# DCASE-REPO/DESED_task

Measured on AMD Instinct MI355X. Metric: 10s-clips/sec CRNN mean-teacher train @batch48, higher is better.
Workload: dtype f32 (fp32 storage and accumulation; the dense contractions of the wide layers run as split-bf16 MFMA, 3 bf16 products per fp32 product, fp32-level accuracy; everything else exact f32)

## Files before the change

### desed_task_amd/_lib.py

```python
import ctypes
import os
import re

_HERE = os.path.dirname(os.path.abspath(__file__))
_HEADER = os.path.join(os.path.dirname(_HERE), "include", "sed_hip.h")
LIB_PATH = os.path.join(_HERE, "libsed_hip.so")

_CTYPES = {"int": ctypes.c_int, "float": ctypes.c_float, "double": ctypes.c_double, "long long": ctypes.c_longlong,
           "unsigned": ctypes.c_uint, "unsigned int": ctypes.c_uint}

ERRORS = {-1: "bad argument", -2: "kernel launch failed", -3: "unsupported configuration"}


def parse_header(path=_HEADER):
    text = open(path).read()
    text = re.sub(r"/\*.*?\*/", "", text, flags=re.S)
    protos = {}
    for m in re.finditer(r"\b(?:int|long long)\s+(sed_\w+)\s*\(([^)]*)\)\s*;", text):
        args = []
        for a in m.group(2).split(","):
            a = a.strip()
            if "*" in a:
                args.append(ctypes.c_void_p)
            else:
                ty = re.sub(r"\bconst\b", "", a).strip()
                ty = ty.rsplit(None, 1)[0].strip()
                args.append(_CTYPES[ty])
        protos[m.group(1)] = args
    return protos


def header_constants(path=_HEADER):
    return {m.group(1): int(m.group(2)) for m in re.finditer(r"^#define\s+(SED_\w+)\s+(\d+)\b", open(path).read(), re.M)}


class _Lib:
    def __init__(self, path, is_emulator=False):
        self.path = path
        self.is_emulator = is_emulator
        import torch
        self._dll = ctypes.CDLL(path)
        self.protos = parse_header()
        for name, argtypes in self.protos.items():
            fn = getattr(self._dll, name)
            fn.argtypes = argtypes
            fn.restype = ctypes.c_longlong if name.endswith("_floats") else ctypes.c_int

    def value(self, name, *args):
        return getattr(self._dll, name)(*args)

    def call(self, name, *args):
        rc = getattr(self._dll, name)(*args)
        if rc != 0:
            raise RuntimeError("%s failed: %s (rc=%d)" % (name, ERRORS.get(rc, "?"), rc))


_lib = None


def get():
    global _lib
    if _lib is None:
        if not os.path.exists(LIB_PATH):
            raise RuntimeError(
                "desed_task_amd: %s is missing -- build it with `python -m desed_task_amd.build` "
                "(hipcc --offload-arch=gfx950).  There is no CPU fallback." % LIB_PATH)
        _lib = _Lib(LIB_PATH)
    return _lib


def use_library(path, is_emulator=True):
    global _lib
    _lib = _Lib(path, is_emulator=is_emulator) if path is not None else None
    return _lib


TUNING_KEYS = {"glu_grid_cap": 0, "glu_bwd128_split": 1, "convb_ck": 2, "convb_mp": 3, "block0_nocenter": 4, "glu_fwd128": 5, "wgrad_narrow": 6, "wgrad_cap": 7, "attn_valu": 8, "wgrad_wide": 9, "gru_lds_kb": 10, "mel_taps_mem": 11, "convb_tpw": 12, "mel_wave": 13, "gemm_ntn": 14, "linear_tiles": 15}


_tuning = {}


def set_tuning(key, value):
    get().call("sed_set_tuning", TUNING_KEYS[key], int(value))
    _tuning[key] = int(value)


def get_tuning(key):
    return _tuning.get(key, 0)


def check_tensor(t, name="tensor"):
    lib = get()
    if lib.is_emulator:
        if t.is_cuda:
            raise RuntimeError("%s: emulator build bound but tensor is on the GPU" % name)
    elif not t.is_cuda:
        raise RuntimeError("%s must live on the MI355X (cuda) device: there is no CPU path" % name)
    if not t.is_contiguous():
        raise RuntimeError("%s must be contiguous" % name)


def stream_ptr(t):
    if t.is_cuda:
        import torch
        return torch.cuda.current_stream(t.device).cuda_stream
    return 0
```

### desed_task_amd/csrc/sed_common.h

```cpp
#pragma once

#ifdef SED_EMU
#include "hip_emu.h"
#else
#include <hip/hip_runtime.h>
#define SED_DYN_SMEM(name) extern __shared__ __attribute__((aligned(16))) char name[]
#define SED_LAUNCH(kern, grid, block, smem, stream, ...) \
    hipLaunchKernelGGL(kern, grid, block, smem, stream, __VA_ARGS__)
typedef float f32x16 __attribute__((ext_vector_type(16)));
typedef float f32x4 __attribute__((ext_vector_type(4)));
typedef short s16x8 __attribute__((ext_vector_type(8)));
#endif

#include <stdint.h>

#define SED_API extern "C" __attribute__((visibility("default")))

#define SED_MAX_SMEM(kern, bytes) \
    (void)hipFuncSetAttribute((const void*)(kern), hipFuncAttributeMaxDynamicSharedMemorySize, (int)(bytes))

__global__ __launch_bounds__(256) static void sed_zero4_kernel(float* p0, int n0, float* p1, int n1, float* p2, int n2, float* p3, int n3) {
    const int i = blockIdx.x * 256 + threadIdx.x;
    if (i < n0) p0[i] = 0.f;
    if (i < n1) p1[i] = 0.f;
    if (i < n2) p2[i] = 0.f;
    if (i < n3) p3[i] = 0.f;
}
static inline void sed_zero4(hipStream_t s, float* p0, int n0, float* p1, int n1, float* p2, int n2, float* p3, int n3) {
    int n = n0 > n1 ? n0 : n1;
    n = n > n2 ? n : n2;
    n = n > n3 ? n : n3;
    if (n <= 0) return;
    SED_LAUNCH(sed_zero4_kernel, dim3((n + 255) / 256), dim3(256), 0, s, p0, n0, p1, n1, p2, n2, p3, n3);
}

#define SED_OK 0
#define SED_ERR_ARG (-1)
#define SED_ERR_LAUNCH (-2)
#define SED_ERR_UNSUPPORTED (-3)

enum { SED_TUNE_GLU_GRID_CAP = 0, SED_TUNE_GLU_BWD128_SPLIT = 1, SED_TUNE_CONVB_CK = 2, SED_TUNE_CONVB_MP = 3, SED_TUNE_B0_NOCENTER = 4, SED_TUNE_GLU_FWD128 = 5, SED_TUNE_WGRAD_NARROW = 6, SED_TUNE_WGRAD_CAP = 7,
       SED_TUNE_ATTN_VALU = 8, SED_TUNE_WGRAD_WIDE = 9, SED_TUNE_GRU_LDS_KB = 10, SED_TUNE_MEL_TAPS_MEM = 11, SED_TUNE_CONVB_TPW = 12, SED_TUNE_MEL_WAVE = 13, SED_TUNE_GEMM_NTN = 14, SED_TUNE_LINEAR_TILES = 15, SED_TUNE_COUNT = 16 };
extern int sed_tuning[SED_TUNE_COUNT];

static inline int sed_check_launch() {
    hipError_t e = hipGetLastError();
    return e == hipSuccess ? SED_OK : SED_ERR_LAUNCH;
}

__device__ __forceinline__ f32x16 mfma32(float a, float b, f32x16 c) {
#ifdef SED_EMU
    return emu_mfma_32x32x2(a, b, c);
#else
    return __builtin_amdgcn_mfma_f32_32x32x2f32(a, b, c, 0, 0, 0);
#endif
}
__device__ __forceinline__ int mfma32_row(int r, int lane) { return (r & 3) + 8 * (r >> 2) + 4 * (lane >> 5); }

__device__ __forceinline__ f32x4 mfma16(float a, float b, f32x4 c) {
#ifdef SED_EMU
    return emu_mfma_16x16x4(a, b, c);
#else
    return __builtin_amdgcn_mfma_f32_16x16x4f32(a, b, c, 0, 0, 0);
#endif
}

__device__ __forceinline__ f32x16 mfma32_bf16(s16x8 a, s16x8 b, f32x16 c) {
#ifdef SED_EMU
    return emu_mfma_32x32x16_bf16(a, b, c);
#else
    typedef __bf16 bf16x8_t __attribute__((ext_vector_type(8)));
    return __builtin_amdgcn_mfma_f32_32x32x16_bf16(__builtin_bit_cast(bf16x8_t, a), __builtin_bit_cast(bf16x8_t, b), c, 0, 0, 0);
#endif
}
__device__ __forceinline__ f32x4 mfma16_bf16(s16x8 a, s16x8 b, f32x4 c) {
#ifdef SED_EMU
    return emu_mfma_16x16x32_bf16(a, b, c);
#else
    typedef __bf16 bf16x8_t __attribute__((ext_vector_type(8)));
    return __builtin_amdgcn_mfma_f32_16x16x32_bf16(__builtin_bit_cast(bf16x8_t, a), __builtin_bit_cast(bf16x8_t, b), c, 0, 0, 0);
#endif
}
__device__ __forceinline__ unsigned short f32_to_bf16(float x) {
    unsigned u = __float_as_uint(x);
    u += 0x7FFFu + ((u >> 16) & 1u);
    return (unsigned short)(u >> 16);
}
__device__ __forceinline__ float bf16_to_f32(unsigned short h) { return __uint_as_float(((unsigned)h) << 16); }
__device__ __forceinline__ void bf16_split(float x, unsigned short& hi, unsigned short& lo) {
    hi = f32_to_bf16(x);
    lo = f32_to_bf16(x - bf16_to_f32(hi));
}

__device__ __forceinline__ float sed_sadd(float a, float b) {
#ifdef SED_EMU
    return a + b;
#else
    float r;
    asm("v_add_f32 %0, %1, %2" : "=v"(r) : "v"(a), "v"(b));
    return r;
#endif
}

__device__ __forceinline__ float sed_sfma(float a, float b, float c) {
#ifdef SED_EMU
    return fmaf(a, b, c);
#else
    float r;
    asm("v_fma_f32 %0, %1, %2, %3" : "=v"(r) : "v"(a), "v"(b), "v"(c));
    return r;
#endif
}

__device__ __forceinline__ void sed_sched_fence() {
#ifndef SED_EMU
    __builtin_amdgcn_sched_barrier(0);
#endif
}

__device__ __forceinline__ unsigned sed_alignbit(unsigned hi, unsigned lo, unsigned shift) {
#ifdef SED_EMU
    return (unsigned)(((((unsigned long long)hi) << 32) | lo) >> shift);
#else
    return __builtin_amdgcn_alignbit(hi, lo, shift);
#endif
// ... 299 lines not shown
```

### desed_task_amd/csrc/sed_conv.hip

```cpp
#include "sed_common.h"

__global__ __launch_bounds__(256) void pack_weights_kernel(const float* __restrict__ W, float* __restrict__ Wf,
                                                           float* __restrict__ Wd, int COUT, int CIN) {
    const int i = blockIdx.x * 256 + threadIdx.x;
    if (i >= COUT * CIN * 9) return;
    const int b = i % 3, a = (i / 3) % 3, ci = (i / 9) % CIN, co = i / (9 * CIN);
    const float w = W[i];
    Wf[((a * 3 + b) * CIN + ci) * COUT + co] = w;
    if (Wd) Wd[(((2 - a) * 3 + (2 - b)) * COUT + co) * CIN + ci] = w;
}
SED_API int sed_conv_pack_weights(const float* W, float* Wf, float* Wd, int COUT, int CIN, void* stream) {
    const int n = COUT * CIN * 9;
    SED_LAUNCH(pack_weights_kernel, dim3((n + 255) / 256), dim3(256), 0, (hipStream_t)stream, W, Wf, Wd, COUT, CIN);
    return sed_check_launch();
}
struct PackJobs {
    const float* W[8];
    float* Wf[8];
    float* Wd[8];
    int cout[8], cin[8], start[9];
    int n;
};
__global__ __launch_bounds__(256) void pack_weights_multi_kernel(PackJobs jobs) {
    const int i = blockIdx.x * 256 + threadIdx.x;
    if (i >= jobs.start[jobs.n]) return;
    int j = 0;
#pragma unroll
    for (int q = 1; q < 8; ++q) j += (q < jobs.n && i >= jobs.start[q]) ? 1 : 0;
    const int e = i - jobs.start[j], COUT = jobs.cout[j], CIN = jobs.cin[j];
    const int b = e % 3, a = (e / 3) % 3, ci = (e / 9) % CIN, co = e / (9 * CIN);
    const float w = jobs.W[j][e];
    jobs.Wf[j][((a * 3 + b) * CIN + ci) * COUT + co] = w;
    if (jobs.Wd[j]) jobs.Wd[j][(((2 - a) * 3 + (2 - b)) * COUT + co) * CIN + ci] = w;
}
SED_API int sed_conv_pack_multi(int n, const void* const* W, void* const* Wf, void* const* Wd, const int* cout, const int* cin,
                                   void* stream) {
    if (n < 1 || n > 8) return SED_ERR_ARG;
    PackJobs jobs;
    int tot = 0;
    for (int j = 0; j < n; ++j) {
        jobs.W[j] = (const float*)W[j]; jobs.Wf[j] = (float*)Wf[j]; jobs.Wd[j] = Wd ? (float*)Wd[j] : nullptr;
        jobs.cout[j] = cout[j]; jobs.cin[j] = cin[j]; jobs.start[j] = tot;
        tot += cout[j] * cin[j] * 9;
    }
    for (int j = n; j < 8; ++j) { jobs.W[j] = nullptr; jobs.Wf[j] = nullptr; jobs.Wd[j] = nullptr; jobs.cout[j] = 0; jobs.cin[j] = 0; jobs.start[j] = tot; }
    jobs.start[n] = tot;
    jobs.start[8] = tot;
    jobs.n = n;
    SED_LAUNCH(pack_weights_multi_kernel, dim3((tot + 255) / 256), dim3(256), 0, (hipStream_t)stream, jobs);
    return sed_check_launch();
}

__global__ __launch_bounds__(1024) void wgrad_reduce_kernel(const float* __restrict__ parts, float* __restrict__ dW, int nparts,
                                                            int COUT, int CIN) {
    __shared__ float4 red[64][16];
    const int tid = threadIdx.x, col = tid & 15, grp = tid >> 4, G = blockDim.x >> 4;
    const int j = blockIdx.x * 64 + 4 * col;
    const int n = 9 * CIN * COUT;
    float4 acc = make_float4(0.f, 0.f, 0.f, 0.f);
    if (j < n) {
#pragma unroll 4
        for (int p = grp; p < nparts; p += G) {
            const float4 v = *(const float4*)(parts + (size_t)p * n + j);
            acc.x += v.x; acc.y += v.y; acc.z += v.z; acc.w += v.w;
        }
    }
    red[grp][col] = acc;
    __syncthreads();
    if (grp == 0 && j < n) {
        for (int g = 1; g < G; ++g) { const float4 v = red[g][col]; acc.x += v.x; acc.y += v.y; acc.z += v.z; acc.w += v.w; }
        const int co = j % COUT, ci = (j / COUT) % CIN, tap = j / (COUT * CIN);
        float* d = dW + ((size_t)co * CIN + ci) * 9 + tap;
        d[0] = acc.x; d[(size_t)CIN * 9] = acc.y; d[(size_t)2 * CIN * 9] = acc.z; d[(size_t)3 * CIN * 9] = acc.w;
    }
}
static inline int wgrad_parts(int CIN, int COUT, int B, int T, int F) {
    if (CIN <= 32) {
        const int TF = F >= 32 ? 32 : F, TR = 128 / TF;
        const int ntiles = B * ((T + TR - 1) / TR) * (F / TF);
        int cap = CIN <= 16 ? 1024 : 512;
        if (sed_tuning[SED_TUNE_WGRAD_CAP] > 0) cap = sed_tuning[SED_TUNE_WGRAD_CAP];
        return ntiles < cap ? ntiles : cap;
    }
    const int ntiles = (B * T * F + 63) / 64;
    return ntiles < 56 ? ntiles : 56;
}
static inline bool wgrad_row_ok(int CIN, int COUT, int F) {
    return F >= 8 && 64 % F == 0 && COUT == 128 && (CIN == 64 || CIN == 128);
}
static inline int wgrad_row_parts(int CIN, int B, int T, int F) {
    const int ntiles = (B * T * F + 63) / 64, cap = CIN == 64 ? 168 : 84;
    return ntiles < cap ? ntiles : cap;
}
SED_API long long sed_conv_wgrad_scratch_floats(int B, int T, int F, int CIN, int COUT) {
    int parts = wgrad_parts(CIN, COUT, B, T, F);
    if (wgrad_row_ok(CIN, COUT, F) && wgrad_row_parts(CIN, B, T, F) > parts) parts = wgrad_row_parts(CIN, B, T, F);
    return (long long)parts * 9 * CIN * COUT;
}

#define CONV_THREADS(COUT) ((COUT) >= 64 ? 512 : 256)

template <int CIN, int COUT, int TF, int MP = 128>
struct ConvCfg {
    static constexpr int TR = MP / TF;
    static constexpr int PW = TF + 2, PH = TR + 2, PP = PW * PH;
    static constexpr int CK = CIN < 32 ? CIN : 32;
    static constexpr int CKP = CK + 1;
    static constexpr int NCH = CIN / CK;
    static constexpr int NT = (COUT + 31) / 32;
    static constexpr int WM = MP / 32;
    static constexpr int THREADS = CONV_THREADS(COUT);
    static constexpr int WN = THREADS / 64 / WM;
    static constexpr int NTW = NT / WN;
    static_assert(NTW >= 1 && NTW * WN == NT, "wave split must tile COUT");
    static constexpr int WCH = CK * COUT;
    static constexpr int PATCH_F = (PP * CKP + 3) & ~3;
    static constexpr int SMEM = (PATCH_F + 2 * WCH) * 4;
};

template <int CIN, int COUT, int TF, bool STATS, int MP = 128>
__global__ __launch_bounds__(CONV_THREADS(COUT)) void conv3x3_kernel(const float* __restrict__ x, const float* __restrict__ Wp,
                                                      const float* __restrict__ bias, float* __restrict__ y,
                                                      float* __restrict__ partial, int B, int T, int F) {
    using Cfg = ConvCfg<CIN, COUT, TF, MP>;
    constexpr int TR = Cfg::TR, PW = Cfg::PW, PP = Cfg::PP, CK = Cfg::CK, CKP = Cfg::CKP, NCH = Cfg::NCH, NT = Cfg::NT,
                  WCH = Cfg::WCH, NTW = Cfg::NTW, THREADS = Cfg::THREADS, WM = Cfg::WM;
    SED_DYN_SMEM(smem);
    float* patch = (float*)smem;
    float* wbuf = patch + Cfg::PATCH_F;
    const int tid = threadIdx.x, lane = tid & 63, w = (tid >> 6) % WM, wn = (tid >> 6) / WM, lo = lane & 31, hi = lane >> 5;
    const int ftiles = F / TF, ttiles = (T + TR - 1) / TR;
    const int bid = blockIdx.x;
    const int ft = bid % ftiles, tt = (bid / ftiles) % ttiles, b = bid / (ftiles * ttiles);
    const int t0 = tt * TR, f0 = ft * TF;
    const int p = 32 * w + lo;
    const int abase = ((p / TF) * PW + (p % TF)) * CKP + hi;

    f32x16 acc[NTW];
#pragma unroll
    for (int nt = 0; nt < NTW; ++nt) acc[nt] = f32x16_zero();

    constexpr int WV = (WCH / 4 + THREADS - 1) / THREADS;
    float4 wreg[WV];

    for (int cc = 0; cc < NCH; ++cc) {
        constexpr int V = CK / 4;
        {
            constexpr int NLD = (PP * V + THREADS - 1) / THREADS;
            float4 ld[NLD];
#pragma unroll
            for (int u = 0; u < NLD; ++u) {
                const int idx = tid + THREADS * u;
                const int pix = idx / V, v = idx - pix * V;
                const int i = pix / PW, j = pix - i * PW;
                const int t = t0 - 1 + i, f = f0 - 1 + j;
                ld[u] = make_float4(0.f, 0.f, 0.f, 0.f);
                if (idx < PP * V && t >= 0 && t < T && f >= 0 && f < F)
                    ld[u] = *(const float4*)(x + (((size_t)b * T + t) * F + f) * CIN + cc * CK + 4 * v);
            }
#pragma unroll
            for (int u = 0; u < NLD; ++u) {
                const int idx = tid + THREADS * u;
                if (idx < PP * V) {
                    const int pix = idx / V, v = idx - pix * V;
                    float* d = patch + pix * CKP + 4 * v;
                    d[0] = ld[u].x; d[1] = ld[u].y; d[2] = ld[u].z; d[3] = ld[u].w;
                }
            }
        }
        {
            const float4* src = (const float4*)(Wp + ((size_t)0 * CIN + cc * CK) * COUT);
#pragma unroll
            for (int i = 0; i < WV; ++i) {
                const int idx = tid + THREADS * i;
                if (idx < WCH / 4) ((float4*)wbuf)[idx] = src[idx];
// ... 340 lines not shown
                const int idx = tid + 256 * u, r = idx / (COUT / 4), v = idx - r * (COUT / 4);
                *(float4*)(ds + r * COUT + 4 * v) = ldy[u];
            }
        }
        __syncthreads();
        constexpr int KS = KT / WK;
#pragma unroll 4
        for (int k = wk * KS; k < (wk + 1) * KS; k += 2) {
            float av[MT];
#pragma unroll
            for (int m = 0; m < MT; ++m) av[m] = (CIN >= 32 || lo < CIN) ? xs[(k + hi) * CIN + m * 32 + lo] : 0.f;
#pragma unroll
            for (int n = 0; n < NTW; ++n) {
                const int co = (wn * NTW + n) * 32 + lo;
                const float bv = (COUT >= 32 || lo < COUT) ? ds[(k + hi) * COUT + co] : 0.f;
#pragma unroll
                for (int m = 0; m < MT; ++m) acc[m][n] = mfma32(av[m], bv, acc[m][n]);
            }
        }
    }
    static_assert(WK == 1, "wide layers: every wave owns its output tiles");
    float* part = dWp + ((size_t)blockIdx.x * 9 + tap) * CIN * COUT;
#pragma unroll
    for (int m = 0; m < MT; ++m)
#pragma unroll
        for (int n = 0; n < NTW; ++n) {
            const int co = (wn * NTW + n) * 32 + lo;
#pragma unroll
            for (int r = 0; r < 16; ++r) {
                const int ci = m * 32 + mfma32_row(r, lane);
                if (ci < CIN && co < COUT) part[(size_t)ci * COUT + co] = acc[m][n][r];
            }
        }
}

template <int CIN, int COUT>
static int launch_wgrad(const float* x, const float* dy, float* dWp, int B, int T, int F, hipStream_t s) {
    using Cfg = WgCfg<CIN, COUT>;
    const int splits = wgrad_parts(CIN, COUT, B, T, F);
    SED_MAX_SMEM((conv_wgrad_kernel<CIN, COUT>), Cfg::SMEM);
    SED_LAUNCH((conv_wgrad_kernel<CIN, COUT>), dim3(splits, 9), dim3(256), Cfg::SMEM, s, x, dy, dWp, B, T, F);
    return sed_check_launch();
}

template <int CIN, int COUT, int NP = 3>
struct WgbCfg {
    static constexpr int PLANES = NP == 1 ? 1 : 2;
    static constexpr int KT = 64, RS = 64;
    static constexpr int MT = CIN / 32, NT = COUT / 32;
    static constexpr int WM = MT >= 4 ? 2 : 1, WN = 4 / WM;
    static constexpr int MTW = MT / WM, NTW = NT / WN;
    static constexpr int NBX = (KT / 4) * (CIN / 4) / 256, NBD = (KT / 4) * (COUT / 4) / 256;
    static constexpr int SMEM = PLANES * (CIN + COUT) * RS * 2;
    static_assert(NBX >= 1 && NBD >= 1 && MTW * WM == MT && NTW * WN == NT, "tile split");
};

template <bool LO = true>
__device__ __forceinline__ void wgb_store_row(float a, float b, float c, float d, unsigned short* __restrict__ hi_row,
                                              unsigned short* __restrict__ lo_row) {
    if constexpr (!LO) {
        *(uint2*)hi_row = make_uint2(bf16_round2(a, b), bf16_round2(c, d));
    } else {
    uint2 h, l;
    bf16_split2(a, b, h.x, l.x);
    bf16_split2(c, d, h.y, l.y);
    *(uint2*)hi_row = h;
    *(uint2*)lo_row = l;
    }
}
template <bool LO = true>
__device__ __forceinline__ void wgb_store_block(const float4 v0, const float4 v1, const float4 v2, const float4 v3,
                                                unsigned short* __restrict__ hi_plane, unsigned short* __restrict__ lo_plane,
                                                int cq, int pq, int RS) {
    const int r0 = 4 * cq, f0 = (r0 ^ cq) & 7;
    const int o0 = r0 * RS + 4 * (pq ^ (2 * f0)), o1 = (r0 + 1) * RS + 4 * (pq ^ (2 * (f0 ^ 1)));
    const int o2 = (r0 + 2) * RS + 4 * (pq ^ (2 * (f0 ^ 2))), o3 = (r0 + 3) * RS + 4 * (pq ^ (2 * (f0 ^ 3)));
    wgb_store_row<LO>(v0.x, v1.x, v2.x, v3.x, hi_plane + o0, lo_plane + o0);
    wgb_store_row<LO>(v0.y, v1.y, v2.y, v3.y, hi_plane + o1, lo_plane + o1);
    wgb_store_row<LO>(v0.z, v1.z, v2.z, v3.z, hi_plane + o2, lo_plane + o2);
    wgb_store_row<LO>(v0.w, v1.w, v2.w, v3.w, hi_plane + o3, lo_plane + o3);
}

template <int CIN, int COUT, class... ONE>
__global__ __launch_bounds__(256) void conv_wgrad_bf16_kernel(const float* __restrict__ x, const float* __restrict__ dy,
                                                              float* __restrict__ dWp, int B, int T, int F) {
    constexpr int NP = sed_np<ONE...>();
    using Cfg = WgbCfg<CIN, COUT, NP>;
    constexpr int KT = Cfg::KT, RS = Cfg::RS, WN = Cfg::WN, MTW = Cfg::MTW, NTW = Cfg::NTW, NBX = Cfg::NBX, NBD = Cfg::NBD;
    SED_DYN_SMEM(smem);
    unsigned short* xh = (unsigned short*)smem;
    unsigned short* xl = xh + (Cfg::PLANES - 1) * CIN * RS;
    unsigned short* dh = xl + CIN * RS;
    unsigned short* dl = dh + (Cfg::PLANES - 1) * COUT * RS;
    const int tid = threadIdx.x, lane = tid & 63, w = tid >> 6, lo = lane & 31, hi = lane >> 5;
    const int wn = w % WN, wm = w / WN;
    const int tap = blockIdx.y, da = tap / 3 - 1, db = tap % 3 - 1;
    const int npix = B * T * F;
    const int ntiles = (npix + KT - 1) / KT;
    const int fsh = 31 - __builtin_clz(F);

    f32x16 acc[MTW][NTW];
#pragma unroll
    for (int m = 0; m < MTW; ++m)
#pragma unroll
        for (int n = 0; n < NTW; ++n) acc[m][n] = f32x16_zero();

    float4 rx[NBX * 4], rd[NBD * 4];
    unsigned okx = 0, okd = 0;
    static_assert(NBX * 4 <= 32 && NBD * 4 <= 32, "validity masks");
    auto load_tile = [&](int tile) {
        const int p0 = tile * KT;
        okx = 0; okd = 0;
#pragma unroll
        for (int u = 0; u < NBX; ++u) {
            const int blk = tid + 256 * u, cq = (blk >> 1) % (CIN / 4), pq = (blk & 1) + 2 * ((blk >> 1) / (CIN / 4));
#pragma unroll
            for (int j = 0; j < 4; ++j) {
                const int p = p0 + 4 * pq + j, pc = p < npix ? p : 0;
                const int f = pc & (F - 1), tt = pc >> fsh, t = tt % T, bb = tt / T;
                const int t2 = t + da, f2 = f + db;
                const bool ok = p < npix && t2 >= 0 && t2 < T && f2 >= 0 && f2 < F;
                okx |= (ok ? 1u : 0u) << (4 * u + j);
                const int t2c = t2 < 0 ? 0 : (t2 >= T ? T - 1 : t2), f2c = f2 < 0 ? 0 : (f2 >= F ? F - 1 : f2);
                rx[4 * u + j] = *(const float4*)(x + (((size_t)bb * T + t2c) * F + f2c) * CIN + 4 * cq);
            }
        }
#pragma unroll
        for (int u = 0; u < NBD; ++u) {
            const int blk = tid + 256 * u, cq = (blk >> 1) % (COUT / 4), pq = (blk & 1) + 2 * ((blk >> 1) / (COUT / 4));
#pragma unroll
            for (int j = 0; j < 4; ++j) {
                const int p = p0 + 4 * pq + j;
                okd |= (p < npix ? 1u : 0u) << (4 * u + j);
                rd[4 * u + j] = *(const float4*)(dy + (size_t)(p < npix ? p : 0) * COUT + 4 * cq);
            }
        }
    };
    auto store_tile = [&]() {
#pragma unroll
        for (int i = 0; i < NBX * 4; ++i) if (!((okx >> i) & 1u)) rx[i] = make_float4(0.f, 0.f, 0.f, 0.f);
#pragma unroll
        for (int i = 0; i < NBD * 4; ++i) if (!((okd >> i) & 1u)) rd[i] = make_float4(0.f, 0.f, 0.f, 0.f);
#pragma unroll
        for (int u = 0; u < NBX; ++u) {
            const int blk = tid + 256 * u;
            wgb_store_block<NP != 1>(rx[4 * u], rx[4 * u + 1], rx[4 * u + 2], rx[4 * u + 3], xh, xl, (blk >> 1) % (CIN / 4),
                            (blk & 1) + 2 * ((blk >> 1) / (CIN / 4)), RS);
        }
#pragma unroll
        for (int u = 0; u < NBD; ++u) {
            const int blk = tid + 256 * u;
            wgb_store_block<NP != 1>(rd[4 * u], rd[4 * u + 1], rd[4 * u + 2], rd[4 * u + 3], dh, dl, (blk >> 1) % (COUT / 4),
                            (blk & 1) + 2 * ((blk >> 1) / (COUT / 4)), RS);
        }
    };

    int tile = blockIdx.x;
    if (tile < ntiles) load_tile(tile);
    for (; tile < ntiles; tile += gridDim.x) {
        __syncthreads();
        store_tile();
        __syncthreads();
        if (tile + (int)gridDim.x < ntiles) load_tile(tile + gridDim.x);
#pragma unroll
        for (int ks = 0; ks < KT / 16; ++ks) {
            const int oct = 2 * ks + hi;
            s16x8 a_hi[MTW], a_lo[MTW];
#pragma unroll
            for (int m = 0; m < MTW; ++m) {
                const int row = (wm * MTW + m) * 32 + lo;
                const int off = row * RS + 8 * (oct ^ ((row ^ (row >> 2)) & 7));
                a_hi[m] = *(const s16x8*)(xh + off);
                if constexpr (NP != 1) a_lo[m] = *(const s16x8*)(xl + off);
            }
#pragma unroll
            for (int n = 0; n < NTW; ++n) {
                const int row = (wn * NTW + n) * 32 + lo;
                const int off = row * RS + 8 * (oct ^ ((row ^ (row >> 2)) & 7));
                const s16x8 b_hi = *(const s16x8*)(dh + off);
                if constexpr (NP == 1) {
#pragma unroll
                    for (int m = 0; m < MTW; ++m) acc[m][n] = mfma32_bf16(a_hi[m], b_hi, acc[m][n]);
                    continue;
                }
                const s16x8 b_lo = *(const s16x8*)(dl + off);
#pragma unroll
                for (int m = 0; m < MTW; ++m) {
                    acc[m][n] = mfma32_bf16(a_lo[m], b_hi, acc[m][n]);
                    acc[m][n] = mfma32_bf16(a_hi[m], b_lo, acc[m][n]);
                    acc[m][n] = mfma32_bf16(a_hi[m], b_hi, acc[m][n]);
                }
            }
        }
    }
    float* part = dWp + ((size_t)blockIdx.x * 9 + tap) * CIN * COUT;
#pragma unroll
    for (int m = 0; m < MTW; ++m)
#pragma unroll
        for (int n = 0; n < NTW; ++n) {
            const int co = (wn * NTW + n) * 32 + lo;
#pragma unroll
            for (int r = 0; r < 16; ++r) part[(size_t)((wm * MTW + m) * 32 + mfma32_row(r, lane)) * COUT + co] = acc[m][n][r];
        }
}

template <int CIN, int COUT, int NP = 3>
static int launch_wgrad_bf16(const float* x, const float* dy, float* dWp, int B, int T, int F, hipStream_t s) {
    using Cfg = WgbCfg<CIN, COUT, NP>;
    const int splits = wgrad_parts(CIN, COUT, B, T, F);
    SED_MAX_SMEM((NP == 1 ? conv_wgrad_bf16_kernel<CIN, COUT, SedOneProduct> : conv_wgrad_bf16_kernel<CIN, COUT>), Cfg::SMEM);
    SED_LAUNCH((NP == 1 ? conv_wgrad_bf16_kernel<CIN, COUT, SedOneProduct> : conv_wgrad_bf16_kernel<CIN, COUT>), dim3(splits, 9), dim3(256), Cfg::SMEM, s, x, dy, dWp, B, T, F);
    return sed_check_launch();
}

template <int CIN, int COUT, int COH, int NP = 3>
struct WgrCfg {
    static constexpr int PLANES = NP == 1 ? 1 : 2;
    static constexpr int KT = 64, RS = 64;
    static constexpr int MT = CIN / 32, NT = COH / 32;
    static constexpr int WM = MT >= 4 ? 2 : 1, WN = 4 / WM;
    static constexpr int MTW = MT / WM, NTW = NT / WN;
    static constexpr int NBX = (KT / 4) * (CIN / 4) / 256, NBD = (KT / 4) * (COH / 4) / 256;
    static constexpr int SMEM = PLANES * (CIN + COH) * RS * 2;
    static_assert(NBX >= 1 && NBD >= 1 && MTW * WM == MT && NTW * WN == NT && MTW * NTW == 2, "tile split");
};
template <int CIN, int COUT, int COH, class... ONE>
__global__ __launch_bounds__(256) void conv_wgrad_bf16_row_kernel(const float* __restrict__ x, const float* __restrict__ dy,
                                                                  float* __restrict__ dWp, int B, int T, int F) {
    constexpr int NP = sed_np<ONE...>();
    using Cfg = WgrCfg<CIN, COUT, COH, NP>;
    constexpr int KT = Cfg::KT, RS = Cfg::RS, WN = Cfg::WN, MTW = Cfg::MTW, NTW = Cfg::NTW, NBX = Cfg::NBX, NBD = Cfg::NBD;
    SED_DYN_SMEM(smem);
    unsigned short* xh = (unsigned short*)smem;
    unsigned short* xl = xh + (Cfg::PLANES - 1) * CIN * RS;
    unsigned short* dh = xl + CIN * RS;
    unsigned short* dl = dh + (Cfg::PLANES - 1) * COH * RS;
    const int lane = threadIdx.x & 63, w = threadIdx.x >> 6;
    int tid = threadIdx.x, lo = lane & 31, hi = lane >> 5;
    const int wn = w % WN, wm = w / WN;
    const int da = (int)blockIdx.y - 1, co0 = blockIdx.z * COH;
    const int npix = B * T * F;
    const int ntiles = (npix + KT - 1) / KT;
    const int fsh = 31 - __builtin_clz(F);

    f32x16 acc[3][MTW][NTW];
#pragma unroll
    for (int t3 = 0; t3 < 3; ++t3)
#pragma unroll
        for (int m = 0; m < MTW; ++m)
#pragma unroll
            for (int n = 0; n < NTW; ++n) acc[t3][m][n] = f32x16_zero();

    float4 rx[NBX * 4], rd[NBD * 4];
    unsigned okm = 0;
    auto load_tile = [&](int tile) {
        const int p0 = tile * KT;
        okm = 0;
#pragma unroll
        for (int u = 0; u < NBX; ++u) {
            const int blk = tid + 256 * u, cq = (blk >> 1) % (CIN / 4), pq = (blk & 1) + 2 * ((blk >> 1) / (CIN / 4));
            const int pb = p0 + 4 * pq, pbc = pb < npix ? pb : 0, tt = pbc >> fsh, t = tt % T, bb = tt / T, t2 = t + da, f = pbc & (F - 1);
            const bool ok = pb < npix && t2 >= 0 && t2 < T;
            okm |= (ok ? 1u : 0u) << u;
            const float* src = x + (((size_t)bb * T + (t2 < 0 ? 0 : (t2 >= T ? T - 1 : t2))) * F + f) * CIN + 4 * cq;
#pragma unroll
            for (int j = 0; j < 4; ++j) rx[4 * u + j] = *(const float4*)(src + (size_t)j * CIN);
        }
#pragma unroll
        for (int u = 0; u < NBD; ++u) {
            const int blk = tid + 256 * u, cq = (blk >> 1) % (COH / 4), pq = (blk & 1) + 2 * ((blk >> 1) / (COH / 4));
            const int pb = p0 + 4 * pq;
            okm |= (pb < npix ? 1u : 0u) << (16 + u);
            const float* src = dy + (size_t)(pb < npix ? pb : 0) * COUT + co0 + 4 * cq;
#pragma unroll
            for (int j = 0; j < 4; ++j) rd[4 * u + j] = *(const float4*)(src + (size_t)j * COUT);
        }
    };
    auto store_tile = [&]() {
#pragma unroll
        for (int u = 0; u < NBX; ++u)
            if (!((okm >> u) & 1u)) {
#pragma unroll
                for (int j = 0; j < 4; ++j) rx[4 * u + j] = make_float4(0.f, 0.f, 0.f, 0.f);
            }
#pragma unroll
        for (int u = 0; u < NBD; ++u)
            if (!((okm >> (16 + u)) & 1u)) {
#pragma unroll
                for (int j = 0; j < 4; ++j) rd[4 * u + j] = make_float4(0.f, 0.f, 0.f, 0.f);
            }
#pragma unroll
        for (int u = 0; u < NBX; ++u) {
            const int blk = tid + 256 * u;
            wgb_store_block<NP != 1>(rx[4 * u], rx[4 * u + 1], rx[4 * u + 2], rx[4 * u + 3], xh, xl, (blk >> 1) % (CIN / 4),
                            (blk & 1) + 2 * ((blk >> 1) / (CIN / 4)), RS);
        }
#pragma unroll
        for (int u = 0; u < NBD; ++u) {
            const int blk = tid + 256 * u;
            wgb_store_block<NP != 1>(rd[4 * u], rd[4 * u + 1], rd[4 * u + 2], rd[4 * u + 3], dh, dl, (blk >> 1) % (COH / 4),
                            (blk & 1) + 2 * ((blk >> 1) / (COH / 4)), RS);
        }
    };
    auto shift_m1 = [](const uint4 c, unsigned prev3) {
        uint4 r;
        r.x = sed_alignbit(c.x, prev3, 16); r.y = sed_alignbit(c.y, c.x, 16); r.z = sed_alignbit(c.z, c.y, 16); r.w = sed_alignbit(c.w, c.z, 16);
        return r;
    };
    auto shift_p1 = [](const uint4 c, unsigned next0) {
        uint4 r;
        r.x = sed_alignbit(c.y, c.x, 16); r.y = sed_alignbit(c.z, c.y, 16); r.z = sed_alignbit(c.w, c.z, 16); r.w = sed_alignbit(next0, c.w, 16);
        return r;
    };

    int tile = blockIdx.x;
    if (tile < ntiles) load_tile(tile);
    for (; tile < ntiles; tile += gridDim.x) {
        sed_opaque(tid); sed_opaque(lo); sed_opaque(hi);
        __syncthreads();
        store_tile();
        __syncthreads();
        if (tile + (int)gridDim.x < ntiles) load_tile(tile + gridDim.x);
#pragma unroll
        for (int ks = 0; ks < KT / 16; ++ks) {
            const int oct = 2 * ks + hi;
            const bool first = ((8 * oct) & (F - 1)) == 0, last = ((8 * oct + 8) & (F - 1)) == 0;
            s16x8 a_hi[3][MTW], a_lo[3][MTW];
#pragma unroll
            for (int m = 0; m < MTW; ++m) {
                const int row = (wm * MTW + m) * 32 + lo, sw = (row ^ (row >> 2)) & 7;
                const int off = row * RS + 8 * (oct ^ sw);
                const int offp = row * RS + 8 * (((oct + 7) & 7) ^ sw) + 6, offn = row * RS + 8 * (((oct + 1) & 7) ^ sw);
                if constexpr (NP == 1) {
                    const uint4 ch = *(const uint4*)(xh + off);
                    const unsigned ph = first ? 0u : *(const unsigned*)(xh + offp), nh = last ? 0u : *(const unsigned*)(xh + offn);
                    a_hi[0][m] = __builtin_bit_cast(s16x8, shift_m1(ch, ph));
                    a_hi[1][m] = __builtin_bit_cast(s16x8, ch);
                    a_hi[2][m] = __builtin_bit_cast(s16x8, shift_p1(ch, nh));
                    continue;
                }
                const uint4 ch = *(const uint4*)(xh + off), cl = *(const uint4*)(xl + off);
                const unsigned ph = first ? 0u : *(const unsigned*)(xh + offp), pl = first ? 0u : *(const unsigned*)(xl + offp);
                const unsigned nh = last ? 0u : *(const unsigned*)(xh + offn), nl = last ? 0u : *(const unsigned*)(xl + offn);
                a_hi[0][m] = __builtin_bit_cast(s16x8, shift_m1(ch, ph)); a_lo[0][m] = __builtin_bit_cast(s16x8, shift_m1(cl, pl));
                a_hi[1][m] = __builtin_bit_cast(s16x8, ch);               a_lo[1][m] = __builtin_bit_cast(s16x8, cl);
                a_hi[2][m] = __builtin_bit_cast(s16x8, shift_p1(ch, nh)); a_lo[2][m] = __builtin_bit_cast(s16x8, shift_p1(cl, nl));
            }
#pragma unroll
            for (int n = 0; n < NTW; ++n) {
                const int row = (wn * NTW + n) * 32 + lo;
                const int off = row * RS + 8 * (oct ^ ((row ^ (row >> 2)) & 7));
                const s16x8 b_hi = *(const s16x8*)(dh + off);
                if constexpr (NP == 1) {
#pragma unroll
                    for (int t3 = 0; t3 < 3; ++t3)
#pragma unroll
                        for (int m = 0; m < MTW; ++m) acc[t3][m][n] = mfma32_bf16(a_hi[t3][m], b_hi, acc[t3][m][n]);
                    continue;
                }
                const s16x8 b_lo = *(const s16x8*)(dl + off);
#pragma unroll
                for (int t3 = 0; t3 < 3; ++t3)
#pragma unroll
                    for (int m = 0; m < MTW; ++m) {
                        acc[t3][m][n] = mfma32_bf16(a_lo[t3][m], b_hi, acc[t3][m][n]);
                        acc[t3][m][n] = mfma32_bf16(a_hi[t3][m], b_lo, acc[t3][m][n]);
                        acc[t3][m][n] = mfma32_bf16(a_hi[t3][m], b_hi, acc[t3][m][n]);
                    }
            }
        }
    }
#pragma unroll
    for (int t3 = 0; t3 < 3; ++t3) {
        float* part = dWp + ((size_t)blockIdx.x * 9 + 3 * (da + 1) + t3) * CIN * COUT;
#pragma unroll
        for (int m = 0; m < MTW; ++m)
#pragma unroll
            for (int n = 0; n < NTW; ++n) {
                const int co = co0 + (wn * NTW + n) * 32 + lo;
#pragma unroll
                for (int r = 0; r < 16; ++r) part[(size_t)((wm * MTW + m) * 32 + mfma32_row(r, lane)) * COUT + co] = acc[t3][m][n][r];
            }
    }
}
template <int CIN, int COUT, int COH, int NP = 3>
static int launch_wgrad_bf16_row(const float* x, const float* dy, float* dWp, int B, int T, int F, int splits, hipStream_t s) {
    using Cfg = WgrCfg<CIN, COUT, COH, NP>;
    SED_MAX_SMEM((NP == 1 ? conv_wgrad_bf16_row_kernel<CIN, COUT, COH, SedOneProduct> : conv_wgrad_bf16_row_kernel<CIN, COUT, COH>), Cfg::SMEM);
    SED_LAUNCH((NP == 1 ? conv_wgrad_bf16_row_kernel<CIN, COUT, COH, SedOneProduct> : conv_wgrad_bf16_row_kernel<CIN, COUT, COH>), dim3(splits, 3, COUT / COH), dim3(256), Cfg::SMEM, s, x, dy, dWp, B, T, F);
    return sed_check_launch();
}

template <int CIN, int COUT, int TF>
struct WgaCfg {
    static constexpr int TR = 128 / TF, PW = TF + 2, PH = TR + 2, PP = PW * PH;
    static constexpr int NT = COUT / 32, WN = NT >= 2 ? 2 : 1, WK = 4 / WN, NTW = NT / WN;
    static constexpr int SMEM = (PP * CIN + 128 * COUT) * 4;
};
template <int CIN, int COUT, int TF>
__global__ __launch_bounds__(256) void conv_wgrad_alltaps_kernel(const float* __restrict__ x, const float* __restrict__ dy,
                                                                 float* __restrict__ dWp, int B, int T, int F) {
    using Cfg = WgaCfg<CIN, COUT, TF>;
    constexpr int TR = Cfg::TR, PW = Cfg::PW, PP = Cfg::PP, WN = Cfg::WN, WK = Cfg::WK, NTW = Cfg::NTW;
    static_assert(CIN <= 32, "narrow layers only");
    SED_DYN_SMEM(smem);
    float* xs = (float*)smem;
    float* ds = xs + PP * CIN;
    const int tid = threadIdx.x, lane = tid & 63, w = tid >> 6, lo = lane & 31, hi = lane >> 5;
    const int wn = w % WN, wk = w / WN;
    const int ftiles = F / TF, ttiles = (T + TR - 1) / TR, ntiles = B * ttiles * ftiles;
    constexpr bool M16 = CIN == 16;
    constexpr int NT16 = COUT / 16, WK16 = 4;
    f32x16 acc[M16 ? 1 : 9][M16 ? 1 : NTW];
    f32x4 acc16[M16 ? 9 : 1][M16 ? NT16 : 1];
#pragma unroll
    for (int tp = 0; tp < (M16 ? 1 : 9); ++tp)
#pragma unroll
        for (int n = 0; n < (M16 ? 1 : NTW); ++n) acc[tp][n] = f32x16_zero();
#pragma unroll
    for (int tp = 0; tp < (M16 ? 9 : 1); ++tp)
#pragma unroll
        for (int n = 0; n < (M16 ? NT16 : 1); ++n) acc16[tp][n] = f32x4{0.f, 0.f, 0.f, 0.f};

    constexpr int NX = (PP * (CIN / 4) + 255) / 256, ND = 128 * (COUT / 4) / 256;
    float4 lx[NX], ldy[ND];
    auto load_tile = [&](int tile_) {
        const int ft = tile_ % ftiles, tt = (tile_ / ftiles) % ttiles, b = tile_ / (ftiles * ttiles);
        const int t0 = tt * TR, f0 = ft * TF;
#pragma unroll
        for (int u = 0; u < NX; ++u) {
            const int idx = tid + 256 * u, pix = idx / (CIN / 4), v = idx - pix * (CIN / 4);
            const int i = pix / PW, j = pix - i * PW;
            const int t = t0 - 1 + i, f = f0 - 1 + j;
            float4 val = make_float4(0.f, 0.f, 0.f, 0.f);
            if (idx < PP * (CIN / 4) && t >= 0 && t < T && f >= 0 && f < F)
                val = *(const float4*)(x + (((size_t)b * T + t) * F + f) * CIN + 4 * v);
            lx[u] = val;
        }
#pragma unroll
        for (int u = 0; u < ND; ++u) {
            const int idx = tid + 256 * u, p = idx / (COUT / 4), v = idx - p * (COUT / 4);
            const int t = t0 + p / TF, f = f0 + p % TF;
            float4 val = make_float4(0.f, 0.f, 0.f, 0.f);
            if (t < T) val = *(const float4*)(dy + (((size_t)b * T + t) * F + f) * COUT + 4 * v);
            ldy[u] = val;
        }
    };
    int tile = blockIdx.x;
    if (tile < ntiles) load_tile(tile);
    for (; tile < ntiles; tile += gridDim.x) {
        __syncthreads();
#pragma unroll
        for (int u = 0; u < NX; ++u) {
            const int idx = tid + 256 * u;
            if (idx < PP * (CIN / 4)) *(float4*)(xs + (idx / (CIN / 4)) * CIN + 4 * (idx % (CIN / 4))) = lx[u];
        }
#pragma unroll
        for (int u = 0; u < ND; ++u) {
            const int idx = tid + 256 * u;
            *(float4*)(ds + (idx / (COUT / 4)) * COUT + 4 * (idx % (COUT / 4))) = ldy[u];
        }
        __syncthreads();
        if (tile + (int)gridDim.x < ntiles) load_tile(tile + gridDim.x);
        if (M16) {
            constexpr int KS16 = 128 / WK16;
            const int i16 = lane & 15, g16 = lane >> 4;
#pragma unroll 2
            for (int k = w * KS16; k < (w + 1) * KS16; k += 4) {
                const int p = k + g16;
                const int pb = (p / TF) * PW + (p % TF);
                float bv16[NT16];
#pragma unroll
// ... 476 lines not shown
```

Before: 16690.

## Run two 256-thread groups per wide wgrad block and reduce accumulators in LDS

The wide-layer bf16 weight-gradient kernels now launch 512 threads, two independent 256-thread groups each with its own LDS planes, processing interleaved tiles. At the end the second group's accumulators are exchanged through LDS and summed by the first group before writing partials. The split counts are halved, so fewer per-split partial slabs need to be written and reduced, and the two groups can overlap loads and MFMA inside one block. In exchange the block uses twice the LDS and a larger block size, which may lower occupancy, and it adds an LDS reduction step. A new tuning knob overrides the split cap.

```diff
diff --git a/desed_task_amd/_lib.py b/desed_task_amd/_lib.py
--- a/desed_task_amd/_lib.py
+++ b/desed_task_amd/_lib.py
@@ -75,7 +75,7 @@
     return _lib
 
 
-TUNING_KEYS = {"glu_grid_cap": 0, "glu_bwd128_split": 1, "convb_ck": 2, "convb_mp": 3, "block0_nocenter": 4, "glu_fwd128": 5, "wgrad_narrow": 6, "wgrad_cap": 7, "attn_valu": 8, "wgrad_wide": 9, "gru_lds_kb": 10, "mel_taps_mem": 11, "convb_tpw": 12, "mel_wave": 13, "gemm_ntn": 14, "linear_tiles": 15}
+TUNING_KEYS = {"glu_grid_cap": 0, "glu_bwd128_split": 1, "convb_ck": 2, "convb_mp": 3, "block0_nocenter": 4, "glu_fwd128": 5, "wgrad_narrow": 6, "wgrad_cap": 7, "attn_valu": 8, "wgrad_wide": 9, "gru_lds_kb": 10, "mel_taps_mem": 11, "convb_tpw": 12, "mel_wave": 13, "gemm_ntn": 14, "linear_tiles": 15, "wgrad_wide_splits": 16}
 
 
 _tuning = {}
diff --git a/desed_task_amd/csrc/sed_common.h b/desed_task_amd/csrc/sed_common.h
--- a/desed_task_amd/csrc/sed_common.h
+++ b/desed_task_amd/csrc/sed_common.h
@@ -40,7 +40,7 @@
 #define SED_ERR_UNSUPPORTED (-3)
 
 enum { SED_TUNE_GLU_GRID_CAP = 0, SED_TUNE_GLU_BWD128_SPLIT = 1, SED_TUNE_CONVB_CK = 2, SED_TUNE_CONVB_MP = 3, SED_TUNE_B0_NOCENTER = 4, SED_TUNE_GLU_FWD128 = 5, SED_TUNE_WGRAD_NARROW = 6, SED_TUNE_WGRAD_CAP = 7,
-       SED_TUNE_ATTN_VALU = 8, SED_TUNE_WGRAD_WIDE = 9, SED_TUNE_GRU_LDS_KB = 10, SED_TUNE_MEL_TAPS_MEM = 11, SED_TUNE_CONVB_TPW = 12, SED_TUNE_MEL_WAVE = 13, SED_TUNE_GEMM_NTN = 14, SED_TUNE_LINEAR_TILES = 15, SED_TUNE_COUNT = 16 };
+       SED_TUNE_ATTN_VALU = 8, SED_TUNE_WGRAD_WIDE = 9, SED_TUNE_GRU_LDS_KB = 10, SED_TUNE_MEL_TAPS_MEM = 11, SED_TUNE_CONVB_TPW = 12, SED_TUNE_MEL_WAVE = 13, SED_TUNE_GEMM_NTN = 14, SED_TUNE_LINEAR_TILES = 15, SED_TUNE_WGRAD_WIDE_SPLITS = 16, SED_TUNE_COUNT = 17 };
 extern int sed_tuning[SED_TUNE_COUNT];
 
 static inline int sed_check_launch() {
diff --git a/desed_task_amd/csrc/sed_conv.hip b/desed_task_amd/csrc/sed_conv.hip
--- a/desed_task_amd/csrc/sed_conv.hip
+++ b/desed_task_amd/csrc/sed_conv.hip
@@ -74,6 +74,17 @@
         d[0] = acc.x; d[(size_t)CIN * 9] = acc.y; d[(size_t)2 * CIN * 9] = acc.z; d[(size_t)3 * CIN * 9] = acc.w;
     }
 }
+#ifndef SED_WGRAD_PINGPONG
+#define SED_WGRAD_PINGPONG 0
+#endif
+#ifndef SED_WGRAD_TAP_WGS
+#define SED_WGRAD_TAP_WGS 28
+#endif
+static inline int wgrad_wide_wgs(int ntiles, int cap) {
+    if (sed_tuning[SED_TUNE_WGRAD_WIDE_SPLITS] > 0) cap = sed_tuning[SED_TUNE_WGRAD_WIDE_SPLITS];
+    const int pairs = (ntiles + 1) / 2;
+    return pairs < cap ? pairs : cap;
+}
 static inline int wgrad_parts(int CIN, int COUT, int B, int T, int F) {
     if (CIN <= 32) {
         const int TF = F >= 32 ? 32 : F, TR = 128 / TF;
@@ -82,15 +93,13 @@
         if (sed_tuning[SED_TUNE_WGRAD_CAP] > 0) cap = sed_tuning[SED_TUNE_WGRAD_CAP];
         return ntiles < cap ? ntiles : cap;
     }
-    const int ntiles = (B * T * F + 63) / 64;
-    return ntiles < 56 ? ntiles : 56;
+    return wgrad_wide_wgs((B * T * F + 63) / 64, SED_WGRAD_TAP_WGS);
 }
 static inline bool wgrad_row_ok(int CIN, int COUT, int F) {
     return F >= 8 && 64 % F == 0 && COUT == 128 && (CIN == 64 || CIN == 128);
 }
 static inline int wgrad_row_parts(int CIN, int B, int T, int F) {
-    const int ntiles = (B * T * F + 63) / 64, cap = CIN == 64 ? 168 : 84;
-    return ntiles < cap ? ntiles : cap;
+    return wgrad_wide_wgs((B * T * F + 63) / 64, CIN == 64 ? 84 : 42);
 }
 SED_API long long sed_conv_wgrad_scratch_floats(int B, int T, int F, int CIN, int COUT) {
     int parts = wgrad_parts(CIN, COUT, B, T, F);
@@ -597,17 +606,18 @@
 }
 
 template <int CIN, int COUT, class... ONE>
-__global__ __launch_bounds__(256) void conv_wgrad_bf16_kernel(const float* __restrict__ x, const float* __restrict__ dy,
+__global__ __launch_bounds__(512) void conv_wgrad_bf16_kernel(const float* __restrict__ x, const float* __restrict__ dy,
                                                               float* __restrict__ dWp, int B, int T, int F) {
     constexpr int NP = sed_np<ONE...>();
     using Cfg = WgbCfg<CIN, COUT, NP>;
     constexpr int KT = Cfg::KT, RS = Cfg::RS, WN = Cfg::WN, MTW = Cfg::MTW, NTW = Cfg::NTW, NBX = Cfg::NBX, NBD = Cfg::NBD;
     SED_DYN_SMEM(smem);
-    unsigned short* xh = (unsigned short*)smem;
+    const int grp = sed_wave_uniform((int)threadIdx.x >> 8);
+    unsigned short* xh = (unsigned short*)(smem + grp * Cfg::SMEM);
     unsigned short* xl = xh + (Cfg::PLANES - 1) * CIN * RS;
     unsigned short* dh = xl + CIN * RS;
     unsigned short* dl = dh + (Cfg::PLANES - 1) * COUT * RS;
-    const int tid = threadIdx.x, lane = tid & 63, w = tid >> 6, lo = lane & 31, hi = lane >> 5;
+    const int tid = threadIdx.x & 255, lane = tid & 63, w = tid >> 6, lo = lane & 31, hi = lane >> 5;
     const int wn = w % WN, wm = w / WN;
     const int tap = blockIdx.y, da = tap / 3 - 1, db = tap % 3 - 1;
     const int npix = B * T * F;
@@ -670,13 +680,18 @@
         }
     };
 
-    int tile = blockIdx.x;
-    if (tile < ntiles) load_tile(tile);
-    for (; tile < ntiles; tile += gridDim.x) {
+    const int stride = 2 * gridDim.x;
+    const int trips = (ntiles - 2 * (int)blockIdx.x + stride - 1) / stride;
+    int tile = 2 * blockIdx.x + grp;
+    load_tile(tile);
+#if SED_WGRAD_PINGPONG
+    if (grp == 1) __syncthreads();
+#endif
+    for (int it = 0; it < trips; ++it, tile += stride) {
         __syncthreads();
         store_tile();
         __syncthreads();
-        if (tile + (int)gridDim.x < ntiles) load_tile(tile + gridDim.x);
+        if (it + 1 < trips) load_tile(tile + stride);
 #pragma unroll
         for (int ks = 0; ks < KT / 16; ++ks) {
             const int oct = 2 * ks + hi;
@@ -708,12 +723,34 @@
             }
         }
     }
+    static_assert(MTW * NTW * 16 * 4 * 256 <= 2 * Cfg::SMEM, "the accumulators of one group fit the planes of two");
+    float4* xch = (float4*)smem;
+#if SED_WGRAD_PINGPONG
+    if (grp == 0) __syncthreads();
+#endif
+    __syncthreads();
+    if (grp == 1) {
+#pragma unroll
+        for (int m = 0; m < MTW; ++m)
+#pragma unroll
+            for (int n = 0; n < NTW; ++n)
+#pragma unroll
+                for (int q = 0; q < 4; ++q)
+                    xch[((m * NTW + n) * 4 + q) * 256 + tid] = make_float4(acc[m][n][4 * q], acc[m][n][4 * q + 1], acc[m][n][4 * q + 2], acc[m][n][4 * q + 3]);
+    }
+    __syncthreads();
+    if (grp != 0) return;
     float* part = dWp + ((size_t)blockIdx.x * 9 + tap) * CIN * COUT;
 #pragma unroll
     for (int m = 0; m < MTW; ++m)
 #pragma unroll
         for (int n = 0; n < NTW; ++n) {
             const int co = (wn * NTW + n) * 32 + lo;
+#pragma unroll
+            for (int q = 0; q < 4; ++q) {
+                const float4 o = xch[((m * NTW + n) * 4 + q) * 256 + tid];
+                acc[m][n][4 * q] += o.x; acc[m][n][4 * q + 1] += o.y; acc[m][n][4 * q + 2] += o.z; acc[m][n][4 * q + 3] += o.w;
+            }
 #pragma unroll
             for (int r = 0; r < 16; ++r) part[(size_t)((wm * MTW + m) * 32 + mfma32_row(r, lane)) * COUT + co] = acc[m][n][r];
         }
@@ -723,8 +760,8 @@
 static int launch_wgrad_bf16(const float* x, const float* dy, float* dWp, int B, int T, int F, hipStream_t s) {
     using Cfg = WgbCfg<CIN, COUT, NP>;
     const int splits = wgrad_parts(CIN, COUT, B, T, F);
-    SED_MAX_SMEM((NP == 1 ? conv_wgrad_bf16_kernel<CIN, COUT, SedOneProduct> : conv_wgrad_bf16_kernel<CIN, COUT>), Cfg::SMEM);
-    SED_LAUNCH((NP == 1 ? conv_wgrad_bf16_kernel<CIN, COUT, SedOneProduct> : conv_wgrad_bf16_kernel<CIN, COUT>), dim3(splits, 9), dim3(256), Cfg::SMEM, s, x, dy, dWp, B, T, F);
+    SED_MAX_SMEM((NP == 1 ? conv_wgrad_bf16_kernel<CIN, COUT, SedOneProduct> : conv_wgrad_bf16_kernel<CIN, COUT>), 2 * Cfg::SMEM);
+    SED_LAUNCH((NP == 1 ? conv_wgrad_bf16_kernel<CIN, COUT, SedOneProduct> : conv_wgrad_bf16_kernel<CIN, COUT>), dim3(splits, 9), dim3(512), 2 * Cfg::SMEM, s, x, dy, dWp, B, T, F);
     return sed_check_launch();
 }
 
@@ -740,18 +777,19 @@
     static_assert(NBX >= 1 && NBD >= 1 && MTW * WM == MT && NTW * WN == NT && MTW * NTW == 2, "tile split");
 };
 template <int CIN, int COUT, int COH, class... ONE>
-__global__ __launch_bounds__(256) void conv_wgrad_bf16_row_kernel(const float* __restrict__ x, const float* __restrict__ dy,
+__global__ __launch_bounds__(512) void conv_wgrad_bf16_row_kernel(const float* __restrict__ x, const float* __restrict__ dy,
                                                                   float* __restrict__ dWp, int B, int T, int F) {
     constexpr int NP = sed_np<ONE...>();
     using Cfg = WgrCfg<CIN, COUT, COH, NP>;
     constexpr int KT = Cfg::KT, RS = Cfg::RS, WN = Cfg::WN, MTW = Cfg::MTW, NTW = Cfg::NTW, NBX = Cfg::NBX, NBD = Cfg::NBD;
     SED_DYN_SMEM(smem);
-    unsigned short* xh = (unsigned short*)smem;
+    const int grp = sed_wave_uniform((int)threadIdx.x >> 8);
+    unsigned short* xh = (unsigned short*)(smem + grp * Cfg::SMEM);
     unsigned short* xl = xh + (Cfg::PLANES - 1) * CIN * RS;
     unsigned short* dh = xl + CIN * RS;
     unsigned short* dl = dh + (Cfg::PLANES - 1) * COH * RS;
-    const int lane = threadIdx.x & 63, w = threadIdx.x >> 6;
-    int tid = threadIdx.x, lo = lane & 31, hi = lane >> 5;
+    const int lane = threadIdx.x & 63, w = (threadIdx.x >> 6) & 3;
+    int tid = threadIdx.x & 255, lo = lane & 31, hi = lane >> 5;
     const int wn = w % WN, wm = w / WN;
     const int da = (int)blockIdx.y - 1, co0 = blockIdx.z * COH;
     const int npix = B * T * F;
@@ -828,14 +866,19 @@
         return r;
     };
 
-    int tile = blockIdx.x;
-    if (tile < ntiles) load_tile(tile);
-    for (; tile < ntiles; tile += gridDim.x) {
+    const int stride = 2 * gridDim.x;
+    const int trips = (ntiles - 2 * (int)blockIdx.x + stride - 1) / stride;
+    int tile = 2 * blockIdx.x + grp;
+    load_tile(tile);
+#if SED_WGRAD_PINGPONG
+    if (grp == 1) __syncthreads();
+#endif
+    for (int it = 0; it < trips; ++it, tile += stride) {
         sed_opaque(tid); sed_opaque(lo); sed_opaque(hi);
         __syncthreads();
         store_tile();
         __syncthreads();
-        if (tile + (int)gridDim.x < ntiles) load_tile(tile + gridDim.x);
+        if (it + 1 < trips) load_tile(tile + stride);
 #pragma unroll
         for (int ks = 0; ks < KT / 16; ++ks) {
             const int oct = 2 * ks + hi;
@@ -885,24 +928,47 @@
             }
         }
     }
+    static_assert(MTW * NTW * 16 * 4 * 256 <= 2 * Cfg::SMEM, "one tap of one group's accumulators fits the planes of two");
+    float4* xch = (float4*)smem;
+#if SED_WGRAD_PINGPONG
+    if (grp == 0) __syncthreads();
+#endif
 #pragma unroll
     for (int t3 = 0; t3 < 3; ++t3) {
-        float* part = dWp + ((size_t)blockIdx.x * 9 + 3 * (da + 1) + t3) * CIN * COUT;
-#pragma unroll
-        for (int m = 0; m < MTW; ++m)
-#pragma unroll
-            for (int n = 0; n < NTW; ++n) {
-                const int co = co0 + (wn * NTW + n) * 32 + lo;
-#pragma unroll
-                for (int r = 0; r < 16; ++r) part[(size_t)((wm * MTW + m) * 32 + mfma32_row(r, lane)) * COUT + co] = acc[t3][m][n][r];
-            }
+        __syncthreads();
+        if (grp == 1) {
+#pragma unroll
+            for (int m = 0; m < MTW; ++m)
+#pragma unroll
+                for (int n = 0; n < NTW; ++n)
+#pragma unroll
+                    for (int q = 0; q < 4; ++q)
+                        xch[((m * NTW + n) * 4 + q) * 256 + tid] = make_float4(acc[t3][m][n][4 * q], acc[t3][m][n][4 * q + 1], acc[t3][m][n][4 * q + 2], acc[t3][m][n][4 * q + 3]);
+        }
+        __syncthreads();
+        if (grp == 0) {
+            float* part = dWp + ((size_t)blockIdx.x * 9 + 3 * (da + 1) + t3) * CIN * COUT;
+#pragma unroll
+            for (int m = 0; m < MTW; ++m)
+#pragma unroll
+                for (int n = 0; n < NTW; ++n) {
+                    const int co = co0 + (wn * NTW + n) * 32 + lo;
+#pragma unroll
+                    for (int q = 0; q < 4; ++q) {
+                        const float4 o = xch[((m * NTW + n) * 4 + q) * 256 + tid];
+                        acc[t3][m][n][4 * q] += o.x; acc[t3][m][n][4 * q + 1] += o.y; acc[t3][m][n][4 * q + 2] += o.z; acc[t3][m][n][4 * q + 3] += o.w;
+                    }
+#pragma unroll
+                    for (int r = 0; r < 16; ++r) part[(size_t)((wm * MTW + m) * 32 + mfma32_row(r, lane)) * COUT + co] = acc[t3][m][n][r];
+                }
+        }
     }
 }
 template <int CIN, int COUT, int COH, int NP = 3>
 static int launch_wgrad_bf16_row(const float* x, const float* dy, float* dWp, int B, int T, int F, int splits, hipStream_t s) {
     using Cfg = WgrCfg<CIN, COUT, COH, NP>;
-    SED_MAX_SMEM((NP == 1 ? conv_wgrad_bf16_row_kernel<CIN, COUT, COH, SedOneProduct> : conv_wgrad_bf16_row_kernel<CIN, COUT, COH>), Cfg::SMEM);
-    SED_LAUNCH((NP == 1 ? conv_wgrad_bf16_row_kernel<CIN, COUT, COH, SedOneProduct> : conv_wgrad_bf16_row_kernel<CIN, COUT, COH>), dim3(splits, 3, COUT / COH), dim3(256), Cfg::SMEM, s, x, dy, dWp, B, T, F);
+    SED_MAX_SMEM((NP == 1 ? conv_wgrad_bf16_row_kernel<CIN, COUT, COH, SedOneProduct> : conv_wgrad_bf16_row_kernel<CIN, COUT, COH>), 2 * Cfg::SMEM);
+    SED_LAUNCH((NP == 1 ? conv_wgrad_bf16_row_kernel<CIN, COUT, COH, SedOneProduct> : conv_wgrad_bf16_row_kernel<CIN, COUT, COH>), dim3(splits, 3, COUT / COH), dim3(512), 2 * Cfg::SMEM, s, x, dy, dWp, B, T, F);
     return sed_check_launch();
 }
 
```

After: 16690 (median of 2 runs). About the same (-0.0%).
